# Julian-Wyatt/AnoDDPM

Hardware: AMD Instinct MI355X
Metric: reverse-diffusion images/sec @256x256 T=1000 simplex (higher is better)
Workload: dtype f32; 1 GPU; 256x256 simplex(8 oct) T=1000 base128 attn16,8 batch4/GPU (BASELINE config 2); per_gpu_batch=4, global_batch=4, T=1000, parallelism=batch-sharded x1 (no data-path collective), output_finite=True

## Files before the change

anoddpm_amd/csrc/attention.hip:

```cpp
#include "common.h"

namespace {

typedef float f32x4 __attribute__((ext_vector_type(4)));

constexpr int AT_LMAX = 1024;
constexpr int AT_WAVES = 8;
constexpr int AT_NT = AT_WAVES * 64;

template <int CHQ>
__global__ __launch_bounds__(AT_NT) void attention_kernel(const anoddpm_attention_args a)
{
    constexpr int CH = CHQ * 16;
    constexpr int QP = CH + 4;
    constexpr int TPW = CHQ >= AT_WAVES ? CHQ / AT_WAVES : 1;
    __shared__ __attribute__((aligned(16))) float lds[16 * (AT_LMAX + 4) + 16 * QP];
    const int L = a.L, SP = L + 4;
    float *S = lds, *Qs = lds + 16 * (AT_LMAX + 4);
    const int tid = threadIdx.x, lane = tid & 63, wave = tid >> 6;
    const int l16 = lane & 15, kq = lane >> 4;
    const int row0 = blockIdx.x * 16, hd = blockIdx.y, b = blockIdx.z;
    const int C3 = 3 * a.heads * CH;
    const float *__restrict__ qkv = a.qkv + (int64_t)b * L * C3 + hd * 3 * CH;
    const int nkt = L >> 4;

    for (int idx = tid; idx < 16 * (CH / 4); idx += AT_NT) {
        const int r = idx / (CH / 4), c4 = idx - r * (CH / 4);
        *reinterpret_cast<f32x4 *>(Qs + r * QP + c4 * 4) = *reinterpret_cast<const f32x4 *>(qkv + (int64_t)(row0 + r) * C3 + c4 * 4);
    }
    constexpr bool DB = CHQ < 32;
    f32x4 kb[DB ? 2 : 1][CHQ];
    auto load_k = [&](f32x4 (&dst)[CHQ], int jt) {
        const float *kp = qkv + (int64_t)(jt * 16 + l16) * C3 + CH + kq * 4;
#pragma unroll
        for (int g = 0; g < CHQ; ++g) dst[g] = *reinterpret_cast<const f32x4 *>(kp + g * 16);
    };
    constexpr int NACC = CHQ >= 32 ? 4 : 1;
    auto score_tile = [&](const f32x4 (&kk)[CHQ], int jt) {
        f32x4 acc[NACC];
#pragma unroll
        for (int c = 0; c < NACC; ++c) acc[c] = f32x4{0.f, 0.f, 0.f, 0.f};
#pragma unroll
        for (int g = 0; g < CHQ; ++g) {
            const f32x4 qa = *reinterpret_cast<const f32x4 *>(Qs + l16 * QP + g * 16 + kq * 4);
#pragma unroll
            for (int e = 0; e < 4; ++e) acc[g % NACC] = __builtin_amdgcn_mfma_f32_16x16x4f32(qa[e], kk[g][e], acc[g % NACC], 0, 0, 0);
        }
        if constexpr (NACC == 4) acc[0] = (acc[0] + acc[1]) + (acc[2] + acc[3]);
#pragma unroll
        for (int r = 0; r < 4; ++r) S[(kq * 4 + r) * SP + jt * 16 + l16] = acc[0][r] * a.scale;
    };
    if (wave < nkt) load_k(kb[0], wave);
    __syncthreads();
    if constexpr (DB) {
        for (int jt = wave; jt < nkt; jt += 2 * AT_WAVES) {
            if (jt + AT_WAVES < nkt) load_k(kb[1], jt + AT_WAVES);
            score_tile(kb[0], jt);
            if (jt + AT_WAVES < nkt) {
                if (jt + 2 * AT_WAVES < nkt) load_k(kb[0], jt + 2 * AT_WAVES);
                score_tile(kb[1], jt + AT_WAVES);
            }
        }
    } else {
        for (int jt = wave; jt < nkt; jt += AT_WAVES) {
            if (jt != wave) load_k(kb[0], jt);
            score_tile(kb[0], jt);
        }
    }
    const int ct0 = wave * TPW;
    const bool pv_active = ct0 < CHQ;
    float vb[2][TPW][4];
    auto load_v = [&](float (&dst)[TPW][4], int kg) {
        const float *vp = qkv + (int64_t)(kg * 16 + kq * 4) * C3 + 2 * CH + ct0 * 16 + l16;
#pragma unroll
        for (int t = 0; t < TPW; ++t)
#pragma unroll
            for (int e = 0; e < 4; ++e) dst[t][e] = vp[(int64_t)e * C3 + t * 16];
    };
    if (pv_active) load_v(vb[0], 0);
    __syncthreads();

    {
        constexpr int TPR = AT_NT / 16;
        const int r = tid / TPR, sub = tid % TPR;
        float *srow = S + r * SP;
        float m = -INFINITY;
        for (int j = sub; j < L; j += TPR) m = fmaxf(m, srow[j]);
#pragma unroll
        for (int o = TPR / 2; o >= 1; o >>= 1) m = fmaxf(m, __shfl_xor(m, o, TPR));
        float sum = 0.f;
        for (int j = sub; j < L; j += TPR) {
            const float e = __expf(srow[j] - m);
            srow[j] = e;
            sum += e;
        }
#pragma unroll
        for (int o = TPR / 2; o >= 1; o >>= 1) sum += __shfl_xor(sum, o, TPR);
        const float inv = 1.0f / sum;
        float *prow = a.probs ? a.probs + (((int64_t)b * a.heads + hd) * L + row0 + r) * L : nullptr;
        for (int j = sub; j < L; j += TPR) {
            const float p = srow[j] * inv;
            srow[j] = p;
            if (prow) prow[j] = p;
        }
    }
    __syncthreads();

    if (!pv_active) return;
    f32x4 oacc[TPW];
#pragma unroll
    for (int t = 0; t < TPW; ++t) oacc[t] = f32x4{0.f, 0.f, 0.f, 0.f};
    auto pv_group = [&](const float (&vv)[TPW][4], int kg) {
        const f32x4 pa = *reinterpret_cast<const f32x4 *>(S + l16 * SP + kg * 16 + kq * 4);
#pragma unroll
        for (int e = 0; e < 4; ++e)
#pragma unroll
            for (int t = 0; t < TPW; ++t) oacc[t] = __builtin_amdgcn_mfma_f32_16x16x4f32(pa[e], vv[t][e], oacc[t], 0, 0, 0);
    };
    for (int kg = 0; kg < nkt; kg += 2) {
        if (kg + 1 < nkt) load_v(vb[1], kg + 1);
        pv_group(vb[0], kg);
        if (kg + 1 < nkt) {
            if (kg + 2 < nkt) load_v(vb[0], kg + 2);
            pv_group(vb[1], kg + 1);
        }
    }
    float *__restrict__ O = a.out + ((int64_t)b * L + row0 + kq * 4) * (a.heads * CH) + hd * CH + ct0 * 16 + l16;
#pragma unroll
    for (int t = 0; t < TPW; ++t)
#pragma unroll
        for (int r = 0; r < 4; ++r) O[(int64_t)r * (a.heads * CH) + t * 16] = oacc[t][r];
}

}

extern "C" int anoddpm_attention(const anoddpm_attention_args *a, void *stream)
{
    ANODDPM_REQUIRE(a && a->qkv && a->out, "attention: null pointer");
    ANODDPM_REQUIRE(a->B >= 1 && a->heads >= 1 && a->B <= 65535 && a->heads <= 65535, "attention: bad batch / head count");
    ANODDPM_REQUIRE(a->L >= 16 && a->L % 16 == 0 && a->L <= AT_LMAX, "attention: L must be a multiple of 16 in [16, 1024]");
    ANODDPM_REQUIRE(a->ch >= 16 && a->ch <= 512 && (a->ch & (a->ch - 1)) == 0, "attention: head width must be a power of two in [16, 512]");
    ANODDPM_REQUIRE(((uintptr_t)a->qkv & 15) == 0, "attention: qkv must be 16-byte aligned");
    const dim3 grid((unsigned)(a->L / 16), (unsigned)a->heads, (unsigned)a->B);
    hipStream_t s = anoddpm::as_stream(stream);
    switch (a->ch / 16) {
        case 1: hipLaunchKernelGGL((attention_kernel<1>), grid, dim3(AT_NT), 0, s, *a); break;
        case 2: hipLaunchKernelGGL((attention_kernel<2>), grid, dim3(AT_NT), 0, s, *a); break;
        case 4: hipLaunchKernelGGL((attention_kernel<4>), grid, dim3(AT_NT), 0, s, *a); break;
        case 8: hipLaunchKernelGGL((attention_kernel<8>), grid, dim3(AT_NT), 0, s, *a); break;
        case 16: hipLaunchKernelGGL((attention_kernel<16>), grid, dim3(AT_NT), 0, s, *a); break;
        default: hipLaunchKernelGGL((attention_kernel<32>), grid, dim3(AT_NT), 0, s, *a); break;
    }
    return anoddpm::check_launch("attention");
}
```

Measured before the change: 0.4513 images/s.

## Use buffer loads with OOB masking and vectorized V column layout in attention PV

Rewrites the PV phase of the attention kernel to load V through raw buffer loads, with out-of-range prefetches masked by an OOB offset instead of branches. Each lane now owns TPW contiguous output columns, so V loads and O stores become 64/128-bit vector accesses. The loop becomes a uniform software pipeline of depth two, and the wave index is made scalar via readfirstlane. The costs are a changed lane-to-column mapping, sched_barriers that constrain the compiler, and new requirements on alignment and per-image size below 2 GiB.

```diff
diff --git a/anoddpm_amd/csrc/attention.hip b/anoddpm_amd/csrc/attention.hip
--- a/anoddpm_amd/csrc/attention.hip
+++ b/anoddpm_amd/csrc/attention.hip
@@ -3,10 +3,17 @@
 namespace {
 
 typedef float f32x4 __attribute__((ext_vector_type(4)));
+typedef float f32x2 __attribute__((ext_vector_type(2)));
 
 constexpr int AT_LMAX = 1024;
 constexpr int AT_WAVES = 8;
+constexpr int AT_OOB = (int)0x80000000u;
 constexpr int AT_NT = AT_WAVES * 64;
+
+__device__ __forceinline__ __amdgpu_buffer_rsrc_t at_rsrc(const float *base)
+{
+    return __builtin_amdgcn_make_buffer_rsrc(const_cast<float *>(base), 0, 0x7ffffffe, 0x00020000);
+}
 
 template <int CHQ>
 __global__ __launch_bounds__(AT_NT) void attention_kernel(const anoddpm_attention_args a)
@@ -17,7 +24,8 @@
     __shared__ __attribute__((aligned(16))) float lds[16 * (AT_LMAX + 4) + 16 * QP];
     const int L = a.L, SP = L + 4;
     float *S = lds, *Qs = lds + 16 * (AT_LMAX + 4);
-    const int tid = threadIdx.x, lane = tid & 63, wave = tid >> 6;
+    const int tid = threadIdx.x, lane = tid & 63;
+    const int wave = __builtin_amdgcn_readfirstlane(tid >> 6);
     const int l16 = lane & 15, kq = lane >> 4;
     const int row0 = blockIdx.x * 16, hd = blockIdx.y, b = blockIdx.z;
     const int C3 = 3 * a.heads * CH;
@@ -67,20 +75,8 @@
             score_tile(kb[0], jt);
         }
     }
-    const int ct0 = wave * TPW;
-    const bool pv_active = ct0 < CHQ;
-    float vb[2][TPW][4];
-    auto load_v = [&](float (&dst)[TPW][4], int kg) {
-        const float *vp = qkv + (int64_t)(kg * 16 + kq * 4) * C3 + 2 * CH + ct0 * 16 + l16;
-#pragma unroll
-        for (int t = 0; t < TPW; ++t)
-#pragma unroll
-            for (int e = 0; e < 4; ++e) dst[t][e] = vp[(int64_t)e * C3 + t * 16];
-    };
-    if (pv_active) load_v(vb[0], 0);
-    __syncthreads();
 
-    {
+    auto softmax_rows = [&]() {
         constexpr int TPR = AT_NT / 16;
         const int r = tid / TPR, sub = tid % TPR;
         float *srow = S + r * SP;
@@ -103,33 +99,73 @@
             srow[j] = p;
             if (prow) prow[j] = p;
         }
-    }
-    __syncthreads();
+    };
 
-    if (!pv_active) return;
+    constexpr int VD = 2;
+    const int ct0 = wave * TPW;
+    const bool pv_active = ct0 < CHQ;
+    const __amdgpu_buffer_rsrc_t rV = at_rsrc(qkv);
+    const unsigned vlane = ((unsigned)(kq * 4) * (unsigned)C3 + (unsigned)(2 * CH + ct0 * 16 + l16 * TPW)) * 4u;
+    float vr[VD][4][TPW];
+    auto load_v = [&](float (&dst)[4][TPW], int kg) {
+        const int vl = kg < nkt ? (int)vlane : AT_OOB;
+#pragma unroll
+        for (int e = 0; e < 4; ++e) {
+            const int so = kg < nkt ? (int)((unsigned)(kg * 16 + e) * (unsigned)C3 * 4u) : 0;
+            if constexpr (TPW == 1) {
+                dst[e][0] = __builtin_bit_cast(float, __builtin_amdgcn_raw_buffer_load_b32(rV, vl, so, 0));
+            } else if constexpr (TPW == 2) {
+                const f32x2 x = __builtin_bit_cast(f32x2, __builtin_amdgcn_raw_buffer_load_b64(rV, vl, so, 0));
+                dst[e][0] = x[0]; dst[e][1] = x[1];
+            } else {
+                const f32x4 x = __builtin_bit_cast(f32x4, __builtin_amdgcn_raw_buffer_load_b128(rV, vl, so, 0));
+#pragma unroll
+                for (int t = 0; t < TPW; ++t) dst[e][t] = x[t];
+            }
+            __builtin_amdgcn_sched_barrier(0);
+        }
+    };
     f32x4 oacc[TPW];
 #pragma unroll
     for (int t = 0; t < TPW; ++t) oacc[t] = f32x4{0.f, 0.f, 0.f, 0.f};
-    auto pv_group = [&](const float (&vv)[TPW][4], int kg) {
+    auto pv_group = [&](const float (&vv)[4][TPW], int kg) {
         const f32x4 pa = *reinterpret_cast<const f32x4 *>(S + l16 * SP + kg * 16 + kq * 4);
 #pragma unroll
         for (int e = 0; e < 4; ++e)
 #pragma unroll
-            for (int t = 0; t < TPW; ++t) oacc[t] = __builtin_amdgcn_mfma_f32_16x16x4f32(pa[e], vv[t][e], oacc[t], 0, 0, 0);
+            for (int t = 0; t < TPW; ++t) oacc[t] = __builtin_amdgcn_mfma_f32_16x16x4f32(pa[e], vv[e][t], oacc[t], 0, 0, 0);
     };
-    for (int kg = 0; kg < nkt; kg += 2) {
-        if (kg + 1 < nkt) load_v(vb[1], kg + 1);
-        pv_group(vb[0], kg);
-        if (kg + 1 < nkt) {
-            if (kg + 2 < nkt) load_v(vb[0], kg + 2);
-            pv_group(vb[1], kg + 1);
+    if (pv_active) {
+#pragma unroll
+        for (int j = 0; j < VD; ++j) load_v(vr[j], j);
+    }
+    __syncthreads();
+    softmax_rows();
+    __syncthreads();
+    if (!pv_active) return;
+    int kg0 = 0;
+    for (; kg0 + VD < nkt; kg0 += VD) {
+#pragma unroll
+        for (int j = 0; j < VD; ++j) {
+            pv_group(vr[j], kg0 + j);
+            load_v(vr[j], kg0 + VD + j);
         }
     }
-    float *__restrict__ O = a.out + ((int64_t)b * L + row0 + kq * 4) * (a.heads * CH) + hd * CH + ct0 * 16 + l16;
 #pragma unroll
-    for (int t = 0; t < TPW; ++t)
+    for (int j = 0; j < VD; ++j)
+        if (kg0 + j < nkt) pv_group(vr[j], kg0 + j);
+    float *__restrict__ O = a.out + ((int64_t)b * L + row0 + kq * 4) * (a.heads * CH) + hd * CH + ct0 * 16 + l16 * TPW;
 #pragma unroll
-        for (int r = 0; r < 4; ++r) O[(int64_t)r * (a.heads * CH) + t * 16] = oacc[t][r];
+    for (int r = 0; r < 4; ++r) {
+        float *o = O + (int64_t)r * (a.heads * CH);
+        if constexpr (TPW == 1) {
+            o[0] = oacc[0][r];
+        } else if constexpr (TPW == 2) {
+            *reinterpret_cast<f32x2 *>(o) = f32x2{oacc[0][r], oacc[1][r]};
+        } else {
+            *reinterpret_cast<f32x4 *>(o) = f32x4{oacc[0][r], oacc[1][r], oacc[2][r], oacc[3][r]};
+        }
+    }
 }
 
 }
@@ -140,7 +176,8 @@
     ANODDPM_REQUIRE(a->B >= 1 && a->heads >= 1 && a->B <= 65535 && a->heads <= 65535, "attention: bad batch / head count");
     ANODDPM_REQUIRE(a->L >= 16 && a->L % 16 == 0 && a->L <= AT_LMAX, "attention: L must be a multiple of 16 in [16, 1024]");
     ANODDPM_REQUIRE(a->ch >= 16 && a->ch <= 512 && (a->ch & (a->ch - 1)) == 0, "attention: head width must be a power of two in [16, 512]");
-    ANODDPM_REQUIRE(((uintptr_t)a->qkv & 15) == 0, "attention: qkv must be 16-byte aligned");
+    ANODDPM_REQUIRE(((uintptr_t)a->qkv & 15) == 0 && ((uintptr_t)a->out & 15) == 0, "attention: qkv and out must be 16-byte aligned");
+    ANODDPM_REQUIRE((int64_t)a->L * 3 * a->heads * a->ch * 4 < ((int64_t)1 << 31), "attention: one image of qkv must stay below 2 GiB (32-bit v offsets)");
     const dim3 grid((unsigned)(a->L / 16), (unsigned)a->heads, (unsigned)a->B);
     hipStream_t s = anoddpm::as_stream(stream);
     switch (a->ch / 16) {
```

New measurement: 0.4527 images/s (median of 6 runs). About the same (+0.3%).
